# EdoardoBotta/RQ-VAE-Recommender

Hardware: AMD Instinct MI355X
Metric: item-embeddings quantized/sec (RQ-VAE fwd+bwd) (higher is better)
Workload: dtype f32 (MLP GEMMs f16x2-emulated)

## Files before the change

### include/rqhip.h

```cpp
#ifndef RQHIP_H
#define RQHIP_H

#include <stddef.h>
#include <stdint.h>

#ifdef __cplusplus
extern "C" {
#endif

#define RQHIP_VERSION 462

#define RQHIP_OK 0
#define RQHIP_EARG (-1)
#define RQHIP_EUNSUPPORTED (-2)
#define RQHIP_EWORKSPACE (-3)

#define RQHIP_MODE_EVAL 0
#define RQHIP_MODE_STE 1
#define RQHIP_MODE_ROTATION 2
#define RQHIP_MODE_GUMBEL 3

typedef void *rqhip_stream_t;

int rqhip_version(void);
// ... 224 lines not shown
    const float *h_mask;
    const float *w_in;
    int w_in_transposed;
    const float *res0;
    float *res0_out;
    const float *codebooks;
    int L, K, mode;
    float beta;
    int64_t *ids;
    float *emb_sum;
    float *loss;
    float *embs_norm;
    const float *w_out;
    int w_out_transposed;
    int out_epilogue;
    const float *out_mask;
    float *out;
    unsigned *out_row_max;
    unsigned *out_col_max;
} rqhip_seam_args;
int rqhip_rq_seam_supported(int D, int H, int L, int K);
int rqhip_rq_seam(const rqhip_seam_args *args, rqhip_stream_t stream);

int rqhip_linear_small_supported(int64_t M, int N, int Kr);
int rqhip_linear_small_plan(int64_t M, int N, int Kr, int *col_blocks, int *waves);
int rqhip_linear_small(const float *a, const float *w, int w_kn, float *out, int64_t M, int N, int Kr, int epilogue, const float *aux,
                       int col_blocks, int waves, rqhip_stream_t stream);

int rqhip_adamw_step(float *const *p, const float *const *g, float *const *m, float *const *v, const int64_t *numel, int n,
                     float *step, unsigned *scratch, float lr, float beta1, float beta2, float eps, float weight_decay,
                     rqhip_stream_t stream);

#define RQHIP_PROF_RQ_FORWARD 1
#define RQHIP_PROF_RQ_BACKWARD 2
#define RQHIP_PROF_GEMM_SPLIT 3
#define RQHIP_PROF_WGRAD 4
#define RQHIP_PROF_MAXIMA 5
#define RQHIP_PROF_IMAGES 6
#define RQHIP_PROF_SEAM 7
#define RQHIP_PROF_LINEAR_SMALL 8
typedef struct {
    int tag;
    float ms;
    double flops, bytes;
} rqhip_profile_record;
int rqhip_profile_enable(int max_records);
// ... 9 lines not shown
```

### rq-vae-recommender_amd/csrc/wgrad.hip

```cpp
#include "rqhip_common.h"

namespace rqhip {

typedef float wg_f32x16 __attribute__((ext_vector_type(16)));
typedef float wg_f32x4 __attribute__((ext_vector_type(4)));
typedef float wg_f32x2 __attribute__((ext_vector_type(2)));

constexpr int kWgChunk = 32;

struct WgradParams {
    const float *g;
    const float *y;
    const float *x;
    float *gm;
    float *out;
    long long M;
    int N, K;
    int nslab_n, nslab_k, msplit;
    long long n_chunks;
    int pow2;
};

template <int V>
struct VecOf;
// ... 256 lines not shown
    pl.cfg = -1;
    if (N % 256 == 0 && K % 256 == 0) { pl.cfg = 0; pl.Nt = 256; pl.Kt = 256; pl.mc = 32; }
    else if (N % 128 == 0 && K % 256 == 0) { pl.cfg = 1; pl.Nt = 128; pl.Kt = 256; pl.mc = 32; }
    else if (N % 256 == 0 && K % 128 == 0) { pl.cfg = 2; pl.Nt = 256; pl.Kt = 128; pl.mc = 32; }
    else if (N % 32 == 0 && K % 128 == 0) { pl.cfg = 3; pl.Nt = 32; pl.Kt = 128; pl.mc = 64; }
    else if (N % 128 == 0 && K % 32 == 0) { pl.cfg = 4; pl.Nt = 128; pl.Kt = 32; pl.mc = 64; }
    if (pl.cfg < 0) return pl;
    pl.nslab_n = N / pl.Nt;
    pl.nslab_k = K / pl.Kt;
    const long long chunks = (M + kWgChunk - 1) / kWgChunk;
    const int slabs = pl.nslab_n * pl.nslab_k;
    long long ms = cu_count() / slabs;
    if (ms < 1) ms = 1;
    if (ms >= 8) ms &= ~7LL;
    if (chunks <= 4) ms = 1;
    if (ms > chunks) ms = chunks > 0 ? chunks : 1;
    pl.msplit = (int)ms;
    pl.pow2 = 1;
    while (pl.pow2 < pl.msplit) pl.pow2 <<= 1;
    pl.lds = (size_t)2 * pl.mc * (pl.Nt + pl.Kt) * sizeof(float);
    return pl;
}

int wgrad_split_cfg(int N, int K);
int launch_wgrad_split_jobs(int n, const float *const *g, const float *const *x, long long M, const int *N, const int *K, float *const *out,
                            int msplit, const unsigned *const *g_max, const unsigned *const *x_max, int half, hipStream_t s);
int launch_wgrad_split(int cfg, const float *g, const float *y, const float *x, long long M, int N, int K, float *gm, float *out,
                       int nslab_n, int nslab_k, int msplit, const unsigned *g_max, const unsigned *x_max, hipStream_t s);

}

using namespace rqhip;

extern "C" size_t rqhip_linear_wgrad_workspace_bytes(int64_t M, int N, int K) {
    if (M <= 0 || N <= 0 || K <= 0) return 0;
    const WgradPlan pl = wgrad_plan(M, N, K);
    if (pl.cfg < 0 || pl.msplit <= 1) return 16;
    return (size_t)pl.msplit * N * K * sizeof(float);
}

extern "C" int rqhip_linear_wgrad_supported(int N, int K) { return wgrad_plan(1 << 20, N, K).cfg >= 0 ? 1 : 0; }

extern "C" int rqhip_linear_wgrad_plan(int64_t M, int N, int K, int *msplit) {
    const WgradPlan pl = wgrad_plan(M, N, K);
    if (msplit) *msplit = pl.cfg < 0 ? 0 : pl.msplit;
    return pl.cfg;
// ... 69 lines not shown
    }
    WgradParams p;
    p.g = g; p.y = y; p.x = x; p.gm = g_masked;
    p.out = pl.msplit > 1 ? reinterpret_cast<float *>(workspace) : dW;
    p.M = M; p.N = N; p.K = K;
    p.nslab_n = pl.nslab_n; p.nslab_k = pl.nslab_k; p.msplit = pl.msplit;
    p.n_chunks = (M + kWgChunk - 1) / kWgChunk;
    p.pow2 = pl.pow2;
    const bool mask = y != nullptr;
    int rc = 0;
    const int scfg = (flags & RQHIP_WGRAD_FP32) ? -1 : wgrad_split_cfg(N, K);
    profile_begin(s, RQHIP_PROF_WGRAD, 2.0 * (double)M * N * K, 4.0 * (double)M * (N * (1 + (y ? 1 : 0) + (g_masked && y ? 1 : 0)) + K));
    if (scfg >= 0 && scfg == pl.cfg) {
        rc = launch_wgrad_split(scfg, g, y, x, M, N, K, g_masked, p.out, pl.nslab_n, pl.nslab_k, pl.msplit, g_col_max, x_col_max, s);
    } else
    switch (pl.cfg) {
        case 0: rc = wgrad_launch<4, 2, 2, 4, 32>(p, pl, mask, s); break;
        case 1: rc = wgrad_launch<4, 1, 1, 8, 32>(p, pl, mask, s); break;
        case 2: rc = wgrad_launch<2, 2, 4, 2, 32>(p, pl, mask, s); break;
        case 3: rc = wgrad_launch<1, 1, 1, 4, 64>(p, pl, mask, s); break;
        default: rc = wgrad_launch<1, 1, 4, 1, 64>(p, pl, mask, s); break;
    }
    if (rc) { profile_end(s); return rc; }
    if (pl.msplit > 1) {
        const size_t nk4 = (size_t)N * K / 4;
        const int tlog = wgrad_reduce_tlog(nk4, pl.pow2);
        const size_t per_wg = (size_t)256 >> tlog;
        hipLaunchKernelGGL(wgrad_reduce_kernel, dim3((unsigned)((nk4 + per_wg - 1) / per_wg)), dim3(256), 0, s,
                           reinterpret_cast<const float *>(workspace), pl.msplit, pl.pow2, tlog, nk4, dW);
        RQ_CHECK_LAUNCH("wgrad_reduce_kernel");
    }
    profile_end(s);
    return RQHIP_OK;
}

static int wgrad_batch_ranges(long long M, const int *N, const int *K, int n, int *half = nullptr) {
    if (n < 2 || n > 4 || M <= 128 || !N || !K) return 0;
    long long tiles = 0;
    int n_full = 0;
    for (int j = 0; j < n; ++j) {
        if (N[j] <= 0 || K[j] <= 0) return 0;
        const int cfg = wgrad_split_cfg(N[j], K[j]);
        if (cfg < 0) return 0;
        n_full += cfg == 0;
        tiles += (long long)(N[j] / (cfg == 1 ? 128 : 256)) * (K[j] / (cfg == 2 ? 128 : 256));
    }
    if (n_full != 0 && n_full != n) return 0;
    if (half) *half = n_full == 0;
    long long ms = cu_count() / tiles;
    if (ms < 1) return 0;
    if (ms >= 8) ms &= ~7LL;
    const long long chunks = (M + kWgChunk - 1) / kWgChunk;
    if (ms > chunks) ms = chunks;
    return (int)ms;
}

// ... 73 lines not shown
```

### rq-vae-recommender_amd/rqhip/_lib.py

```python
from __future__ import annotations

import ctypes as C
import os
import subprocess

import torch

_CSRC = os.path.join(os.path.dirname(os.path.dirname(os.path.abspath(__file__))), "csrc")
SO_PATH = os.path.join(_CSRC, "librqhip.so")

MODE_EVAL, MODE_STE, MODE_ROTATION, MODE_GUMBEL = 0, 1, 2, 3
FWD_SCAN_FP32, FWD_SCAN_VALU, FWD_NO_COOP_TAIL = 0x1, 0x2, 0x10
WGRAD_FP32 = 0x1
BWD_CBGRAD_MATRIX = 0x1
SPLIT_F16X2, SPLIT_BF16X3 = 0, 1
EPI_STORE, EPI_RELU, EPI_RECON, EPI_MASK = 0, 1, 2, 3
PROF_TAGS = {1: "rq_forward", 2: "rq_backward", 3: "gemm_split", 4: "wgrad", 5: "maxima", 6: "weight_images", 7: "rq_seam", 8: "linear_small"}


class ImageJob(C.Structure):
    _fields_ = [("w", C.c_void_p), ("rows", C.c_int), ("cols", C.c_int), ("transpose", C.c_int), ("arith", C.c_int),
                ("image", C.c_void_p), ("image_bytes", C.c_size_t)]


# ... 98 lines not shown
    "rqhip_linear_wgrad_workspace_bytes": (_sz, [_i64, _int, _int]),
    "rqhip_linear_wgrad": (_int, [_vp, _vp, _vp, _i64, _int, _int, _vp, _vp, _vp, _sz, _vp]),
    "rqhip_linear_wgrad_ex": (_int, [_vp, _vp, _vp, _i64, _int, _int, _vp, _vp, _vp, _sz, C.c_uint, _vp]),
    "rqhip_linear_wgrad_f16": (_int, [_vp, _vp, _vp, _i64, _int, _int, _vp, _vp, _vp, _vp, _vp, _sz, _vp]),
    "rqhip_linear_wgrad_f16_batch_plan": (_int, [_i64, C.POINTER(_int), C.POINTER(_int), _int]),
    "rqhip_linear_wgrad_f16_batch_workspace_bytes": (_sz, [_i64, C.POINTER(_int), C.POINTER(_int), _int]),
    "rqhip_linear_wgrad_f16_batch": (_int, [C.POINTER(WgradJob), _int, _i64, _vp, _sz, _vp]),
    "rqhip_linear_wgrad_jobs_supported": (_int, [_int, _int]),
    "rqhip_linear_wgrad_jobs": (_int, [_vp, _vp, _vp, C.POINTER(_int), C.POINTER(_int), _int, _i64, _vp]),
    "rqhip_gemm_split_supported": (_int, [_int, _int]),
    "rqhip_weight_image_bytes": (_sz, [_int, _int, _int]),
    "rqhip_weight_images": (_int, [C.POINTER(ImageJob), _int, _vp]),
    "rqhip_maxima": (_int, [_vp, _vp, _vp, _i64, _int, _vp, _vp, _vp]),
    "rqhip_gemm_split_ex": (_int, [C.POINTER(GemmArgs), _vp]),
    "rqhip_weight_planes_bytes": (_sz, [_int, _int]),
    "rqhip_weight_planes": (_int, [_vp, _int, _int, _int, _vp, _sz, _vp]),
    "rqhip_gemm_split": (_int, [_vp, _i64, _int, _vp, _int, _int, _vp, _vp]),
    "rqhip_gemm_split_recon_workspace_bytes": (_sz, [_i64, _int]),
    "rqhip_gemm_split_recon": (_int, [_vp, _i64, _int, _vp, _int, _vp, _f32, _vp, _vp, _vp, _sz, _vp]),
    "rqhip_recon_rescale_rows": (_int, [_vp, _i64, _int, _f32, _vp, _vp]),
    "rqhip_recon_rescale_rows_ex": (_int, [_vp, _i64, _int, _f32, _vp, _vp, _int, _vp, _vp]),
    "rqhip_rq_seam_supported": (_int, [_int, _int, _int, _int]),
    "rqhip_rq_seam": (_int, [C.POINTER(SeamArgs), _vp]),
    "rqhip_linear_small_supported": (_int, [_i64, _int, _int]),
    "rqhip_linear_small_plan": (_int, [_i64, _int, _int, C.POINTER(_int), C.POINTER(_int)]),
    "rqhip_linear_small": (_int, [_vp, _vp, _int, _vp, _i64, _int, _int, _int, _vp, _int, _int, _vp]),
    "rqhip_adamw_step": (_int, [_vp, _vp, _vp, _vp, _vp, _int, _vp, _vp, _f32, _f32, _f32, _f32, _f32, _vp]),
    "rqhip_profile_enable": (_int, [_int]),
    "rqhip_profile_select": (_int, [C.c_uint]),
    "rqhip_profile_read": (_int, [C.POINTER(_f32), _int, C.POINTER(_int)]),
    "rqhip_profile_read_tagged": (_int, [C.POINTER(ProfileRecord), _int, C.POINTER(_int)]),
}


class RqHipError(RuntimeError):
    pass


def build(force: bool = False) -> str:
    cmd = ["make", "-C", _CSRC, "-j8"] + (["-B"] if force else [])
    proc = subprocess.run(cmd, stdout=subprocess.PIPE, stderr=subprocess.STDOUT, text=True)
    if proc.returncode != 0:
        raise RqHipError("building librqhip.so failed:\n" + proc.stdout[-4000:])
    return SO_PATH


_lib = None


def load(path: str) -> C.CDLL:
    global _lib
    if not os.path.exists(path):
        raise RqHipError(
            f"{path} not found: build it with `python __graft_entry__.py` or `make -C {_CSRC}`. "
            "The HIP extension is the product path; there is no CPU fallback.")
    handle = C.CDLL(path)
    for name, (res, args) in SIGNATURES.items():
        fn = getattr(handle, name)
        fn.restype, fn.argtypes = res, args
    _lib = handle
    return handle


def lib() -> C.CDLL:
    return _lib if _lib is not None else load(SO_PATH)


def check(rc: int, what: str) -> None:
    if rc != 0:
        msg = lib().rqhip_last_error().decode("utf-8", "replace")
        kind = "HIP error" if rc > 0 else "argument error"
        raise RqHipError(f"{what}: {kind} {rc}: {msg}")
```

### rq-vae-recommender_amd/rqhip/autograd.py

```python
from __future__ import annotations

from typing import Optional

import torch
from torch import Tensor

from . import ops


def _dense(g: Optional[Tensor]) -> Optional[Tensor]:
    if g is None:
        return None
    return g.contiguous()


class RqStackFunction(torch.autograd.Function):

    @staticmethod
    def forward(ctx, res0: Tensor, codebooks: Tensor, mode: int, beta: float, want_levels: bool, grad_sink=None):
        out = ops.rq_forward(res0, codebooks, mode, beta, want_embs=want_levels, want_residuals=want_levels)
        ctx.set_materialize_grads(False)
        ctx.save_for_backward(res0, codebooks, out.ids)
        ctx.mode, ctx.beta, ctx.want_levels, ctx.grad_sink = mode, beta, want_levels, grad_sink
        embs = out.embs if want_levels else res0.new_empty((0,))
# ... 36 lines not shown
        cols = both[:ops.SEAM_H] if want_scales else None
        ctx.bwd_cols = both[ops.SEAM_H:] if (want_scales and torch.is_grad_enabled()) else None
        r = ops.rq_seam(h=h, w_in=w_in.detach(), codebooks=codebooks.detach(), mode=mode, beta=beta, w_out=w_out.detach(),
                        epilogue=_lib.EPI_RELU, want_row_max=want_scales, col_max_out=cols)
        ctx.set_materialize_grads(False)
        ctx.save_for_backward(h, w_in, codebooks, w_out, r.res0, r.ids, r.emb_sum, r.out)
        ctx.mode, ctx.beta, ctx.grad_sink, ctx.want_scales = mode, beta, grad_sink, want_scales
        rmax = r.out_row_max if want_scales else h.new_empty((0,), dtype=torch.int32)
        cmax = cols if want_scales else h.new_empty((0,), dtype=torch.int32)
        ctx.mark_non_differentiable(r.ids, r.embs_norm, rmax, cmax)
        return r.ids, r.loss, r.embs_norm, r.out, rmax, cmax

    @staticmethod
    def backward(ctx, _g_ids, g_loss, _g_norm, g_d, _g_rmax=None, _g_cmax=None):
        from . import linear as _lin
        from .dist import claim_grad_sink
        h, w_in, codebooks, w_out, res0, ids, emb_sum, d = ctx.saved_tensors
        need_h, need_win, need_cb, need_wout = ctx.needs_input_grad[:4]
        g_d, g_loss = _dense(g_d), _dense(g_loss)
        B = h.shape[0]
        jobs = _lin.wgrad_jobs_ok(B, [tuple(w_out.shape), tuple(w_in.shape)])
        pending = []
        gw_out = gw_in = None
        g_es = None
        if g_d is not None:
            g_dm = None
            if need_wout:
                if jobs:
                    g_dm = torch.ops.aten.threshold_backward(g_d, d, 0.0)
                    pending.append(_lin.WgradJob(w_out, g_dm, emb_sum, None, None, claim_grad_sink(w_out)))
                else:
                    sink = claim_grad_sink(w_out)
                    gw, gp, _ = _lin.weight_grad(g_d, d, emb_sum, w_out, out=sink, want_masked=False)
                    gw_out = gw.view_as(gw) if sink is not None else gw
                    g_dm = gp if (gp is not None and gp is not g_d) else None
            if need_h or need_win or need_cb:
                g_es = (_lin.chain_input_grad(g_dm, w_out)[0] if g_dm is not None
                        else _lin.chain_input_grad(g_d, w_out, g_mask=d)[0])
        g_res0 = g_cb = None
        if need_h or need_win or need_cb:
            sink = ctx.grad_sink
            out_cb = None
            if need_cb and sink is not None and tuple(sink.view.shape) == tuple(codebooks.shape) and all(
                    p.grad is None and getattr(p, "_rq_sink_epoch", -1) != sink.owner.epoch for p in sink.params):
                out_cb = sink.view
                for p in sink.params:
                    p._rq_sink_epoch = sink.owner.epoch
            g_res0, g_cb = ops.rq_backward(res0, codebooks, ctx.mode, ctx.beta, ids, g_embsum=g_es, g_loss=g_loss,
                                           need_res0=need_h or need_win, need_codebooks=need_cb, out_g_codebooks=out_cb,
                                           cbgrad=ops.cbgrad_default())
            if out_cb is not None and g_cb is not None:
                g_cb = g_cb.view_as(g_cb)
        g_h = None
        if g_res0 is not None and need_win:
            if jobs:
                pending.append(_lin.WgradJob(w_in, g_res0, h, None, None, claim_grad_sink(w_in)))
            else:
                sink = claim_grad_sink(w_in)
                gw, _, _ = _lin.weight_grad(g_res0, None, h, w_in, out=sink)
                gw_in = gw.view_as(gw) if sink is not None else gw
        for j, gw in zip(pending, _lin.launch_wgrads(pending)):
            gw = gw.view_as(gw) if j.sink is not None else gw
            if j.w is w_out:
                gw_out = gw
            else:
                gw_in = gw
        if g_res0 is not None and need_h:
            cols = None
            if ctx.want_scales:
                cols, ctx.bwd_cols = ctx.bwd_cols, None
                if cols is None:
                    cols = _lin.zeros_i32(ops.SEAM_H, h.device)
            g_h, sc = _lin.chain_input_grad(g_res0, w_in, out_mask=h, want_rows=ctx.want_scales, col_out=cols)
            _lin.handoff_grad(g_h, sc if ctx.want_scales else _lin.Scales())
        return g_h, gw_in, g_cb, gw_out, None, None, None, None

# ... 168 lines not shown
```

### rq-vae-recommender_amd/rqhip/linear.py

```python
from enum import IntEnum
from typing import List, NamedTuple, Optional, Sequence, Tuple

import torch
from torch import Tensor

from . import _lib, ops

SPLIT_MIN_ROWS = 4096
_SPLIT_GEMMS = True
_ARITH = ops.F16X2
_FP32 = -1
_ARITH_NAMES = {"f16x2": ops.F16X2, "bf16x3": ops.BF16X3, "fp32": _FP32}


def use_split_gemms(on: bool = True) -> bool:
    global _SPLIT_GEMMS
    before, _SPLIT_GEMMS = _SPLIT_GEMMS, bool(on)
    return before


def use_arith(name: str) -> str:
    global _ARITH
    before = arith_name()
    _ARITH = _ARITH_NAMES[name]
# ... 267 lines not shown
    return _CHAIN


def chain_forward(x: Tensor, w: Tensor, relu: bool, want_rows: bool = False, col_out: Optional[Tensor] = None):
    x = x if x.is_contiguous() else x.contiguous()
    if tuple(w.shape) == (CHAIN_D, CHAIN_H):
        assert not relu
        return ops.rq_seam(h=x, w_in=w.detach()).res0, Scales()
    r = ops.rq_seam(res0=x, w_out=w.detach(), epilogue=_lib.EPI_RELU if relu else _lib.EPI_STORE, want_row_max=want_rows and f16(),
                    col_max_out=col_out if f16() else None)
    return r.out, Scales(r.out_row_max, col_out if f16() else None)


def chain_input_grad(g: Tensor, w: Tensor, *, g_mask: Optional[Tensor] = None, out_mask: Optional[Tensor] = None, want_rows: bool = False,
                     col_out: Optional[Tensor] = None):
    g = g if g.is_contiguous() else g.contiguous()
    if tuple(w.shape) == (CHAIN_H, CHAIN_D):
        assert out_mask is None
        return ops.rq_seam(h=g, h_mask=g_mask, w_in=w.detach(), w_in_transposed=True).res0, Scales()
    assert g_mask is None
    r = ops.rq_seam(res0=g, w_out=w.detach(), w_out_transposed=True, epilogue=_lib.EPI_MASK if out_mask is not None else _lib.EPI_STORE,
                    out_mask=out_mask, want_row_max=want_rows and f16(), col_max_out=col_out if f16() else None)
    return r.out, Scales(r.out_row_max, col_out if f16() else None)


_SMALL = True


def use_small_kernels(on: bool = True) -> bool:
    global _SMALL
    before, _SMALL = _SMALL, bool(on)
    return before


def small_forward(x: Tensor, w: Tensor, relu: bool) -> Tensor:
    return ops.linear_small(x, w.detach(), epilogue=_lib.EPI_RELU if relu else _lib.EPI_STORE)


def small_input_grad(g: Tensor, w: Tensor, below: Optional[Tensor] = None) -> Tensor:
    return ops.linear_small(g, w.detach(), w_kn=True, epilogue=_lib.EPI_MASK if below is not None else _lib.EPI_STORE, aux=below)


class Route(IntEnum):
    NONE = 0
    LIBRARY = 1
    SPLIT = 2
# ... 147 lines not shown
```

### rq-vae-recommender_amd/rqhip/ops.py

```python
from __future__ import annotations

import ctypes as C
from typing import NamedTuple, Optional

import torch
from torch import Tensor

from . import _lib
from ._lib import MODE_EVAL, MODE_GUMBEL, MODE_ROTATION, MODE_STE, RqHipError, check


def _need_gpu(*tensors: Optional[Tensor]) -> torch.device:
    dev = None
    for t in tensors:
        if t is None:
            continue
        if not t.is_cuda:
            raise RqHipError(
                "rqhip ops need ROCm device tensors (got a %s tensor); the HIP kernels are the only "
                "implementation of this path -- there is no CPU fallback." % t.device.type)
        if dev is None:
            dev = t.device
        elif t.device != dev:
            raise RqHipError(f"tensors on different devices: {dev} vs {t.device}")
# ... 141 lines not shown
    if epilogue == _lib.EPI_MASK and (out_mask is None or tuple(out_mask.shape) != (B, H)):
        raise RqHipError("rq_seam: EPI_MASK needs out_mask [B,128]")
    if col_max_out is not None and (col_max_out.dtype != torch.int32 or col_max_out.numel() != H or not col_max_out.is_contiguous()):
        raise RqHipError("rq_seam: col_max_out must be a contiguous int32 [128] tensor (zeroed by the caller)")
    with torch.cuda.device(dev):
        f = lambda *shape: torch.empty(shape, dtype=torch.float32, device=dev)
        a = _lib.SeamArgs()
        a.B, a.D, a.H = B, D, H
        a.h, a.h_mask, a.w_in, a.w_in_transposed = _ptr(h), _ptr(h_mask), _ptr(w_in), int(bool(w_in_transposed))
        r0 = f(B, D) if (h is not None and want_res0) else None
        a.res0, a.res0_out = _ptr(res0) if h is None else None, _ptr(r0)
        ids = torch.empty((L, B), dtype=torch.int64, device=dev) if L > 0 else None
        es = f(B, D) if (L > 0 and want_emb_sum) else None
        loss = f(B) if (L > 0 and want_loss) else None
        norms = f(B, L) if (L > 0 and want_norm) else None
        a.codebooks, a.L, a.K, a.mode, a.beta = _ptr(codebooks), L, K, int(mode), float(beta)
        a.ids, a.emb_sum, a.loss, a.embs_norm = _ptr(ids), _ptr(es), _ptr(loss), _ptr(norms)
        out = f(B, H) if w_out is not None else None
        rmx = torch.empty((H // 32, B), dtype=torch.int32, device=dev) if (w_out is not None and want_row_max) else None
        a.w_out, a.w_out_transposed, a.out_epilogue = _ptr(w_out), int(bool(w_out_transposed)), int(epilogue)
        a.out_mask, a.out, a.out_row_max, a.out_col_max = _ptr(out_mask), _ptr(out), _ptr(rmx), _ptr(col_max_out if w_out is not None else None)
        check(_lib.lib().rqhip_rq_seam(C.byref(a), _stream()), "rqhip_rq_seam")
    return RqSeamOut(r0, ids, es, loss, norms, out, rmx, col_max_out if w_out is not None else None)


def rq_forward(res0: Tensor, codebooks: Tensor, mode: int, beta: float, *, want_embs: bool = True,
               want_residuals: bool = True, want_emb_sum: bool = True, want_loss: bool = True,
               want_norm: bool = True, want_margin: bool = False, scan: str = "auto",
               coop_tail: bool = True) -> RqForwardOut:
    _need_gpu(res0, codebooks)
    res0, codebooks = _f32c(res0, "res0"), _f32c(codebooks, "codebooks")
    if res0.dim() != 2 or codebooks.dim() != 3 or codebooks.shape[2] != res0.shape[1]:
        raise RqHipError(f"shape mismatch: res0 {tuple(res0.shape)}, codebooks {tuple(codebooks.shape)}")
    B, D = res0.shape
    L, K, _ = codebooks.shape
    dev = res0.device
    with torch.cuda.device(dev):
        l = _lib.lib()
        ids = torch.empty((L, B), dtype=torch.int64, device=dev)
        f = lambda *s: torch.empty(s, dtype=torch.float32, device=dev)
        embs = f(L, B, D) if want_embs else None
        residuals = f(L, B, D) if want_residuals else None
        emb_sum = f(B, D) if want_emb_sum else None
        loss = f(B) if want_loss else None
        norm = f(B, L) if want_norm else None
        margin = f(L, B) if want_margin else None
# ... 1042 lines not shown
```

Baseline: 41.00 million.

## Fuse seam backward input-grad and weight-grad GEMMs into single-pass kernels

Adds two HIP kernels for the RQ seam backward. One computes the decoder-side weight gradient and the input gradient g_es in a single pass over g_d, d and emb_sum. The other does the same for the encoder-side linear, producing g_h, dW_in, and the row/column maxima used for f16 scaling. The reductions of both weight-gradient partials are deferred and merged into one pair-reduce launch, removing separate activation reads and several kernel launches. The cost is fixed 128x32 shape specialisation, fp32 MFMA instead of the split-precision paths, and extra LDS pressure.

```diff
diff --git a/include/rqhip.h b/include/rqhip.h
--- a/include/rqhip.h
+++ b/include/rqhip.h
@@ -270,6 +270,12 @@
 int rqhip_rq_seam_supported(int D, int H, int L, int K);
 int rqhip_rq_seam(const rqhip_seam_args *args, rqhip_stream_t stream);
 
+int rqhip_seam_bwd_supported(int D, int H);
+int rqhip_seam_bwd_out(const float *g_d, const float *d, const float *emb_sum, const float *w_out, int64_t M, float *g_es, float *dW_out,
+                       void *workspace, size_t workspace_bytes, int defer_reduce, rqhip_stream_t stream);
+int rqhip_seam_bwd_in(const float *g_res0, const float *h, const float *w_in, int64_t M, float *g_h, unsigned *row_max, unsigned *col_max,
+                      float *dW_in, void *workspace, size_t workspace_bytes, const void *out_workspace, float *dW_out, rqhip_stream_t stream);
+
 int rqhip_linear_small_supported(int64_t M, int N, int Kr);
 int rqhip_linear_small_plan(int64_t M, int N, int Kr, int *col_blocks, int *waves);
 int rqhip_linear_small(const float *a, const float *w, int w_kn, float *out, int64_t M, int N, int Kr, int epilogue, const float *aux,
diff --git a/rq-vae-recommender_amd/csrc/seam_backward.hip b/rq-vae-recommender_amd/csrc/seam_backward.hip
--- /dev/null
+++ b/rq-vae-recommender_amd/csrc/seam_backward.hip
@@ -0,0 +1,411 @@
+#include <type_traits>
+
+#include "rqhip_common.h"
+
+namespace rqhip {
+
+typedef float sb_f32x16 __attribute__((ext_vector_type(16)));
+typedef float sb_f32x4 __attribute__((ext_vector_type(4)));
+
+constexpr int kSbH = 128, kSbD = 32;
+constexpr int kSbNT = 256;
+constexpr int kSbMC = 128;
+constexpr int kSbWS = kSbH + 4;
+constexpr int kSbNS = kSbD + 4;
+constexpr int kSbChunk = 32;
+constexpr int kSbImg = kSbH * kSbD;
+
+int launch_wgrad_reduce(const float *part, int msplit, int N, int K, float *dW, hipStream_t s);
+int launch_wgrad_reduce_pair(const float *part0, int N0, int K0, float *dW0, const float *part1, int N1, int K1, float *dW1, int msplit,
+                             hipStream_t s);
+
+struct SeamBwdParams {
+    const float *g;
+    const float *y;
+    const float *x;
+    const float *w;
+    float *gx;
+    unsigned *row_max;
+    unsigned *col_max;
+    float *part;
+    long long M, n_chunks;
+    int msplit;
+};
+
+__device__ __forceinline__ void sb_stage_weight(float *img, const float *__restrict__ w, int n_out) {
+    constexpr int kPer = kSbImg / kSbNT;
+    float v[kPer];
+#pragma unroll
+    for (int u = 0; u < kPer; ++u) v[u] = w[threadIdx.x + u * kSbNT];
+#pragma unroll
+    for (int u = 0; u < kPer; ++u) {
+        const int e = threadIdx.x + u * kSbNT;
+        const int n = e % n_out, d = e / n_out;
+        const int kk = d >> 1, hh = d & 1;
+        img[(((kk >> 2) * 2 + hh) * n_out + n) * 4 + (kk & 3)] = v[u];
+    }
+}
+
+__device__ __forceinline__ void sb_row_range(const SeamBwdParams &p, long long &r_begin, long long &r_end) {
+    const int split = blockIdx.x;
+    r_begin = (p.n_chunks * split / p.msplit) * kSbChunk;
+    r_end = (p.n_chunks * (split + 1) / p.msplit) * kSbChunk;
+    if (r_end > p.M) r_end = p.M;
+}
+
+__global__ __launch_bounds__(kSbNT) void seam_bwd_out_kernel(const SeamBwdParams p) {
+    constexpr int G4 = kSbMC * kSbH / 4 / kSbNT, X4 = kSbMC * kSbD / 4 / kSbNT;
+    extern __shared__ __attribute__((aligned(16))) char sb_smem[];
+    float *sG = reinterpret_cast<float *>(sb_smem);
+    float *sX = sG + kSbMC * kSbWS;
+    float *img = sX + kSbMC * kSbD;
+
+    const int tid = threadIdx.x, lane = tid & 63, wave = tid >> 6, il = lane & 31, h = lane >> 5;
+    long long r_begin, r_end;
+    sb_row_range(p, r_begin, r_end);
+    const long long n_stage = (r_end - r_begin + kSbMC - 1) / kSbMC;
+
+    sb_f32x4 rg[G4], ry[G4], rx[X4];
+    const sb_f32x4 zero4 = {0.f, 0.f, 0.f, 0.f};
+    auto fetch = [&](long long c) {
+        const long long row0 = r_begin + c * kSbMC;
+#pragma unroll
+        for (int q = 0; q < G4; ++q) {
+            const int f = tid + q * kSbNT;
+            const long long row = row0 + f / (kSbH / 4);
+            const bool ok = row < r_end;
+            const size_t off = (size_t)(ok ? row : 0) * kSbH + 4 * (f % (kSbH / 4));
+            rg[q] = ok ? *reinterpret_cast<const sb_f32x4 *>(p.g + off) : zero4;
+            ry[q] = ok ? *reinterpret_cast<const sb_f32x4 *>(p.y + off) : zero4;
+        }
+#pragma unroll
+        for (int q = 0; q < X4; ++q) {
+            const int f = tid + q * kSbNT;
+            const long long row = row0 + f / (kSbD / 4);
+            const bool ok = row < r_end;
+            rx[q] = ok ? *reinterpret_cast<const sb_f32x4 *>(p.x + (size_t)(ok ? row : 0) * kSbD + 4 * (f % (kSbD / 4))) : zero4;
+        }
+    };
+    auto stash = [&]() {
+#pragma unroll
+        for (int q = 0; q < G4; ++q) {
+            const int f = tid + q * kSbNT;
+            sb_f32x4 v = rg[q];
+            v.x = ry[q].x <= 0.0f ? 0.0f : v.x;
+            v.y = ry[q].y <= 0.0f ? 0.0f : v.y;
+            v.z = ry[q].z <= 0.0f ? 0.0f : v.z;
+            v.w = ry[q].w <= 0.0f ? 0.0f : v.w;
+            *reinterpret_cast<sb_f32x4 *>(sG + (f / (kSbH / 4)) * kSbWS + 4 * (f % (kSbH / 4))) = v;
+        }
+#pragma unroll
+        for (int q = 0; q < X4; ++q) {
+            const int f = tid + q * kSbNT;
+            *reinterpret_cast<sb_f32x4 *>(sX + 4 * f) = rx[q];
+        }
+    };
+
+    sb_f32x16 acc;
+#pragma unroll
+    for (int r = 0; r < 16; ++r) acc[r] = 0.0f;
+
+    if (n_stage > 0) fetch(0);
+    sb_stage_weight(img, p.w, kSbD);
+    if (n_stage > 0) stash();
+    __syncthreads();
+    for (long long c = 0; c < n_stage; ++c) {
+        const bool more = c + 1 < n_stage;
+        if (more) fetch(c + 1);
+        const long long row0 = r_begin + c * kSbMC;
+        const int rows = (int)(r_end - row0 < kSbMC ? r_end - row0 : kSbMC);
+        const float *gA = sG + wave * 32 + il, *xB = sX + il;
+        auto stage = [&](auto full) {
+            constexpr bool FULL = decltype(full)::value;
+#pragma unroll
+            for (int half = 0; half < kSbMC / 64; ++half) {
+                if (!FULL && half * 64 >= rows) break;
+#pragma unroll
+                for (int s = 0; s < 32; ++s) {
+                    const int r = half * 64 + 2 * s + h;
+                    acc = __builtin_amdgcn_mfma_f32_32x32x2f32(gA[r * kSbWS], xB[r * kSbD], acc, 0, 0, 0);
+                }
+            }
+            if (FULL || wave * 32 < rows) {
+                const sb_f32x4 *rowp = reinterpret_cast<const sb_f32x4 *>(sG + (wave * 32 + il) * kSbWS);
+                float x[kSbH / 2];
+#pragma unroll
+                for (int j = 0; j < kSbH / 4; ++j) {
+                    const sb_f32x4 v = rowp[j];
+                    x[2 * j] = h ? v.y : v.x;
+                    x[2 * j + 1] = h ? v.w : v.z;
+                }
+                const sb_f32x4 *img4 = reinterpret_cast<const sb_f32x4 *>(img);
+                sb_f32x16 ge;
+#pragma unroll
+                for (int r = 0; r < 16; ++r) ge[r] = 0.0f;
+#pragma unroll
+                for (int q = 0; q < kSbH / 8; ++q) {
+                    const sb_f32x4 a = img4[(q * 2 + h) * kSbD + il];
+#pragma unroll
+                    for (int i = 0; i < 4; ++i) ge = __builtin_amdgcn_mfma_f32_32x32x2f32(a[i], x[4 * q + i], ge, 0, 0, 0);
+                }
+                const long long row = row0 + wave * 32 + il;
+                if (FULL || row < r_end) {
+                    sb_f32x4 *dst = reinterpret_cast<sb_f32x4 *>(p.gx + (size_t)row * kSbD + 4 * h);
+#pragma unroll
+                    for (int g = 0; g < 4; ++g) dst[2 * g] = sb_f32x4{ge[4 * g], ge[4 * g + 1], ge[4 * g + 2], ge[4 * g + 3]};
+                }
+            }
+        };
+        if (rows == kSbMC) stage(std::true_type{});
+        else stage(std::false_type{});
+        __syncthreads();
+        if (more) stash();
+        __syncthreads();
+    }
+    float *dst = p.part + (size_t)blockIdx.x * kSbH * kSbD;
+#pragma unroll
+    for (int r = 0; r < 16; ++r) dst[(size_t)(wave * 32 + 8 * (r >> 2) + 4 * h + (r & 3)) * kSbD + il] = acc[r];
+}
+
+__global__ __launch_bounds__(kSbNT) void seam_bwd_in_kernel(const SeamBwdParams p) {
+    constexpr int H4 = kSbMC * kSbH / 4 / kSbNT, N4 = kSbMC * kSbD / 4 / kSbNT;
+    extern __shared__ __attribute__((aligned(16))) char sb_smem[];
+    float *sH = reinterpret_cast<float *>(sb_smem);
+    float *sN = sH + kSbMC * kSbWS;
+    float *img = sN + kSbMC * kSbNS;
+    unsigned *colmax_s = reinterpret_cast<unsigned *>(img + kSbImg);
+
+    const int tid = threadIdx.x, lane = tid & 63, wave = tid >> 6, il = lane & 31, h = lane >> 5;
+    long long r_begin, r_end;
+    sb_row_range(p, r_begin, r_end);
+    const long long n_stage = (r_end - r_begin + kSbMC - 1) / kSbMC;
+
+    sb_f32x4 rh[H4], rn[N4];
+    const sb_f32x4 zero4 = {0.f, 0.f, 0.f, 0.f};
+    auto fetch = [&](long long c) {
+        const long long row0 = r_begin + c * kSbMC;
+#pragma unroll
+        for (int q = 0; q < H4; ++q) {
+            const int f = tid + q * kSbNT;
+            const long long row = row0 + f / (kSbH / 4);
+            const bool ok = row < r_end;
+            rh[q] = ok ? *reinterpret_cast<const sb_f32x4 *>(p.y + (size_t)(ok ? row : 0) * kSbH + 4 * (f % (kSbH / 4))) : zero4;
+        }
+#pragma unroll
+        for (int q = 0; q < N4; ++q) {
+            const int f = tid + q * kSbNT;
+            const long long row = row0 + f / (kSbD / 4);
+            const bool ok = row < r_end;
+            rn[q] = ok ? *reinterpret_cast<const sb_f32x4 *>(p.g + (size_t)(ok ? row : 0) * kSbD + 4 * (f % (kSbD / 4))) : zero4;
+        }
+    };
+    unsigned cmx[4] = {0u, 0u, 0u, 0u};
+    auto swap_stage = [&](long long c, bool write_out, bool stash) {
+        const long long row0 = r_begin + c * kSbMC;
+#pragma unroll
+        for (int q = 0; q < H4; ++q) {
+            const int f = tid + q * kSbNT;
+            const int r = f / (kSbH / 4), c4 = f % (kSbH / 4);
+            sb_f32x4 *slot = reinterpret_cast<sb_f32x4 *>(sH + r * kSbWS + 4 * c4);
+            if (write_out && row0 + r < r_end) {
+                const sb_f32x4 v = *slot;
+                *reinterpret_cast<sb_f32x4 *>(p.gx + (size_t)(row0 + r) * kSbH + 4 * c4) = v;
+                const float vc[4] = {v.x, v.y, v.z, v.w};
+#pragma unroll
+                for (int j = 0; j < 4; ++j) {
+                    const unsigned bits = __builtin_bit_cast(unsigned, vc[j]) & 0x7fffffffu;
+                    cmx[j] = bits > cmx[j] ? bits : cmx[j];
+                }
+            }
+            if (stash) *slot = rh[q];
+        }
+        if (stash) {
+#pragma unroll
+            for (int q = 0; q < N4; ++q) {
+                const int f = tid + q * kSbNT;
+                *reinterpret_cast<sb_f32x4 *>(sN + (f / (kSbD / 4)) * kSbNS + 4 * (f % (kSbD / 4))) = rn[q];
+            }
+        }
+    };
+
+    sb_f32x16 acc;
+#pragma unroll
+    for (int r = 0; r < 16; ++r) acc[r] = 0.0f;
+
+    if (n_stage > 0) fetch(0);
+    if (tid < kSbH) colmax_s[tid] = 0u;
+    sb_stage_weight(img, p.w, kSbH);
+    if (n_stage > 0) swap_stage(0, false, true);
+    __syncthreads();
+    const int blk = wave;
+    for (long long c = 0; c < n_stage; ++c) {
+        const bool more = c + 1 < n_stage;
+        if (more) fetch(c + 1);
+        const long long row0 = r_begin + c * kSbMC;
+        const int rows = (int)(r_end - row0 < kSbMC ? r_end - row0 : kSbMC);
+        const float *gA = sN + il, *xB = sH + blk * 32 + il;
+        const sb_f32x4 *img4 = reinterpret_cast<const sb_f32x4 *>(img);
+        auto tiles = [&](auto full) {
+            constexpr bool FULL = decltype(full)::value;
+#pragma unroll
+            for (int t = 0; t < kSbMC / 32; ++t) {
+                if (!FULL && (t & ~1) * 32 >= rows) break;
+#pragma unroll
+                for (int s = 0; s < 16; ++s) {
+                    const int r = t * 32 + 2 * s + h;
+                    acc = __builtin_amdgcn_mfma_f32_32x32x2f32(gA[r * kSbNS], xB[r * kSbWS], acc, 0, 0, 0);
+                }
+                if (!FULL && t * 32 >= rows) continue;
+                const sb_f32x4 *rowp = reinterpret_cast<const sb_f32x4 *>(sN + (t * 32 + il) * kSbNS);
+                float es[kSbD / 2];
+#pragma unroll
+                for (int j = 0; j < kSbD / 4; ++j) {
+                    const sb_f32x4 v = rowp[j];
+                    es[2 * j] = h ? v.y : v.x;
+                    es[2 * j + 1] = h ? v.w : v.z;
+                }
+                sb_f32x16 gh;
+#pragma unroll
+                for (int r = 0; r < 16; ++r) gh[r] = 0.0f;
+#pragma unroll
+                for (int q = 0; q < kSbD / 8; ++q) {
+                    const sb_f32x4 a = img4[(q * 2 + h) * kSbH + 32 * blk + il];
+#pragma unroll
+                    for (int i = 0; i < 4; ++i) gh = __builtin_amdgcn_mfma_f32_32x32x2f32(a[i], es[4 * q + i], gh, 0, 0, 0);
+                }
+                const long long row = row0 + t * 32 + il;
+                const bool row_ok = FULL || row < r_end;
+                float *slot = sH + (t * 32 + il) * kSbWS + 32 * blk + 4 * h;
+                unsigned rmx = 0u;
+#pragma unroll
+                for (int g = 0; g < 4; ++g) {
+                    sb_f32x4 v = {gh[4 * g], gh[4 * g + 1], gh[4 * g + 2], gh[4 * g + 3]};
+                    const sb_f32x4 m = *reinterpret_cast<const sb_f32x4 *>(slot + 8 * g);
+                    v.x = m.x <= 0.0f ? 0.0f : v.x; v.y = m.y <= 0.0f ? 0.0f : v.y;
+                    v.z = m.z <= 0.0f ? 0.0f : v.z; v.w = m.w <= 0.0f ? 0.0f : v.w;
+                    *reinterpret_cast<sb_f32x4 *>(slot + 8 * g) = v;
+                    const float vc[4] = {v.x, v.y, v.z, v.w};
+#pragma unroll
+                    for (int cc = 0; cc < 4; ++cc) {
+                        const unsigned bits = __builtin_bit_cast(unsigned, vc[cc]) & 0x7fffffffu;
+                        rmx = bits > rmx ? bits : rmx;
+                    }
+                }
+                if (p.row_max) {
+                    const unsigned o = (unsigned)shfl_xor32((int)rmx);
+                    rmx = o > rmx ? o : rmx;
+                    if (row_ok && h == 0) p.row_max[(size_t)blk * p.M + row] = rmx;
+                }
+            }
+        };
+        if (rows == kSbMC) tiles(std::true_type{});
+        else tiles(std::false_type{});
+        __syncthreads();
+        swap_stage(c, true, more);
+        __syncthreads();
+    }
+    float *dst = p.part + (size_t)blockIdx.x * kSbH * kSbD;
+#pragma unroll
+    for (int r = 0; r < 16; ++r) dst[(size_t)(8 * (r >> 2) + 4 * h + (r & 3)) * kSbH + 32 * blk + il] = acc[r];
+    if (p.col_max) {
+#pragma unroll
+        for (int j = 0; j < 4; ++j)
+            if (cmx[j]) atomicMax(&colmax_s[4 * (tid & 31) + j], cmx[j]);
+        __syncthreads();
+        if (tid < kSbH && colmax_s[tid]) atomicMax(p.col_max + tid, colmax_s[tid]);
+    }
+}
+
+constexpr size_t kSbOutLds = (size_t)(kSbMC * kSbWS + kSbMC * kSbD + kSbImg) * sizeof(float);
+constexpr size_t kSbInLds = (size_t)(kSbMC * kSbWS + kSbMC * kSbNS + kSbImg + kSbH) * sizeof(float);
+
+static bool sb_al16(const void *q) { return (reinterpret_cast<uintptr_t>(q) & 15u) == 0; }
+
+static int sb_ranges(int64_t M, int N, int K) {
+    int msplit = 0;
+    const int cfg = rqhip_linear_wgrad_plan(M, N, K, &msplit);
+    return (cfg == 3 || cfg == 4) ? msplit : 0;
+}
+
+}
+
+using namespace rqhip;
+
+extern "C" int rqhip_seam_bwd_supported(int D, int H) { return (D == kSbD && H == kSbH) ? 1 : 0; }
+
+static size_t sb_workspace_bytes(int64_t M) { return rqhip_linear_wgrad_workspace_bytes(M, kSbH, kSbD); }
+
+extern "C" int rqhip_seam_bwd_out(const float *g_d, const float *d, const float *emb_sum, const float *w_out, int64_t M, float *g_es,
+                                  float *dW_out, void *workspace, size_t workspace_bytes, int defer_reduce, rqhip_stream_t stream) {
+    if (M < 4096 || !g_d || !d || !emb_sum || !w_out || !g_es || !dW_out) {
+        set_error("seam_bwd_out: null pointer or fewer than 4096 rows (M = %lld)", (long long)M);
+        return M >= 0 && M < 4096 ? RQHIP_EUNSUPPORTED : RQHIP_EARG;
+    }
+    if (!sb_al16(g_d) || !sb_al16(d) || !sb_al16(emb_sum) || !sb_al16(w_out) || !sb_al16(g_es) || !sb_al16(dW_out) || !sb_al16(workspace)) {
+        set_error("seam_bwd_out: pointers must be 16-byte aligned");
+        return RQHIP_EARG;
+    }
+    const int msplit = sb_ranges(M, kSbH, kSbD);
+    if (msplit < 1) {
+        set_error("seam_bwd_out: no weight-gradient plan for 128 x 32");
+        return RQHIP_EUNSUPPORTED;
+    }
+    if (msplit > 1 && (!workspace || workspace_bytes < sb_workspace_bytes(M))) {
+        set_error("seam_bwd_out: workspace too small (rqhip_linear_wgrad_workspace_bytes(M, 128, 32))");
+        return RQHIP_EWORKSPACE;
+    }
+    hipStream_t s = reinterpret_cast<hipStream_t>(stream);
+    SeamBwdParams p;
+    p.g = g_d; p.y = d; p.x = emb_sum; p.w = w_out; p.gx = g_es; p.row_max = nullptr; p.col_max = nullptr;
+    p.part = msplit > 1 ? reinterpret_cast<float *>(workspace) : dW_out;
+    p.M = M; p.n_chunks = (M + kSbChunk - 1) / kSbChunk; p.msplit = msplit;
+    static LdsGrant grant;
+    RQ_RETURN_IF_HIP(grant.ensure(reinterpret_cast<const void *>(seam_bwd_out_kernel), 160 * 1024));
+    profile_begin(s, RQHIP_PROF_SEAM, 4.0 * (double)M * kSbH * kSbD, 4.0 * (double)M * (2 * kSbH + 2 * kSbD));
+    hipLaunchKernelGGL(seam_bwd_out_kernel, dim3(msplit), dim3(kSbNT), kSbOutLds, s, p);
+    profile_end(s);
+    RQ_CHECK_LAUNCH("seam_bwd_out_kernel");
+    if (msplit > 1 && !defer_reduce) return launch_wgrad_reduce(p.part, msplit, kSbH, kSbD, dW_out, s);
+    return RQHIP_OK;
+}
+
+extern "C" int rqhip_seam_bwd_in(const float *g_res0, const float *h, const float *w_in, int64_t M, float *g_h, unsigned *row_max,
+                                 unsigned *col_max, float *dW_in, void *workspace, size_t workspace_bytes, const void *out_workspace,
+                                 float *dW_out, rqhip_stream_t stream) {
+    if (M < 4096 || !g_res0 || !h || !w_in || !g_h || !dW_in || ((out_workspace != nullptr) != (dW_out != nullptr))) {
+        set_error("seam_bwd_in: null pointer, fewer than 4096 rows (M = %lld), or only one of out_workspace / dW_out", (long long)M);
+        return M >= 0 && M < 4096 ? RQHIP_EUNSUPPORTED : RQHIP_EARG;
+    }
+    if (!sb_al16(g_res0) || !sb_al16(h) || !sb_al16(w_in) || !sb_al16(g_h) || !sb_al16(dW_in) || !sb_al16(workspace) ||
+        !sb_al16(out_workspace) || !sb_al16(dW_out)) {
+        set_error("seam_bwd_in: pointers must be 16-byte aligned");
+        return RQHIP_EARG;
+    }
+    const int msplit = sb_ranges(M, kSbD, kSbH);
+    if (msplit < 1 || (out_workspace && sb_ranges(M, kSbH, kSbD) != msplit)) {
+        set_error("seam_bwd_in: no weight-gradient plan for 32 x 128 (or another number of row ranges than the deferred 128 x 32 blocks)");
+        return RQHIP_EUNSUPPORTED;
+    }
+    if (msplit > 1 && (!workspace || workspace_bytes < sb_workspace_bytes(M))) {
+        set_error("seam_bwd_in: workspace too small (rqhip_linear_wgrad_workspace_bytes(M, 128, 32))");
+        return RQHIP_EWORKSPACE;
+    }
+    hipStream_t s = reinterpret_cast<hipStream_t>(stream);
+    SeamBwdParams p;
+    p.g = g_res0; p.y = h; p.x = nullptr; p.w = w_in; p.gx = g_h; p.row_max = row_max; p.col_max = col_max;
+    p.part = msplit > 1 ? reinterpret_cast<float *>(workspace) : dW_in;
+    p.M = M; p.n_chunks = (M + kSbChunk - 1) / kSbChunk; p.msplit = msplit;
+    static LdsGrant grant;
+    RQ_RETURN_IF_HIP(grant.ensure(reinterpret_cast<const void *>(seam_bwd_in_kernel), 160 * 1024));
+    profile_begin(s, RQHIP_PROF_SEAM, 4.0 * (double)M * kSbH * kSbD, 4.0 * (double)M * (2 * kSbH + kSbD + (row_max ? 4 : 0)));
+    hipLaunchKernelGGL(seam_bwd_in_kernel, dim3(msplit), dim3(kSbNT), kSbInLds, s, p);
+    profile_end(s);
+    RQ_CHECK_LAUNCH("seam_bwd_in_kernel");
+    if (msplit > 1) {
+        if (out_workspace)
+            return launch_wgrad_reduce_pair(reinterpret_cast<const float *>(out_workspace), kSbH, kSbD, dW_out, p.part, kSbD, kSbH, dW_in,
+                                            msplit, s);
+        return launch_wgrad_reduce(p.part, msplit, kSbD, kSbH, dW_in, s);
+    }
+    return RQHIP_OK;
+}
diff --git a/rq-vae-recommender_amd/csrc/wgrad.hip b/rq-vae-recommender_amd/csrc/wgrad.hip
--- a/rq-vae-recommender_amd/csrc/wgrad.hip
+++ b/rq-vae-recommender_amd/csrc/wgrad.hip
@@ -302,6 +302,47 @@
     return pl;
 }
 
+static int wgrad_reduce_go(const float *part, int msplit, int N, int K, float *dW, hipStream_t s) {
+    int pow2 = 1;
+    while (pow2 < msplit) pow2 <<= 1;
+    const size_t nk4 = (size_t)N * K / 4;
+    const int tlog = wgrad_reduce_tlog(nk4, pow2);
+    const size_t per_wg = (size_t)256 >> tlog;
+    hipLaunchKernelGGL(wgrad_reduce_kernel, dim3((unsigned)((nk4 + per_wg - 1) / per_wg)), dim3(256), 0, s, part, msplit, pow2, tlog, nk4, dW);
+    RQ_CHECK_LAUNCH("wgrad_reduce_kernel");
+    return 0;
+}
+
+int launch_wgrad_reduce(const float *part, int msplit, int N, int K, float *dW, hipStream_t s) {
+    profile_begin(s, RQHIP_PROF_WGRAD, 0.0, 4.0 * (double)N * K * (msplit + 1));
+    const int rc = wgrad_reduce_go(part, msplit, N, K, dW, s);
+    profile_end(s);
+    return rc;
+}
+
+int launch_wgrad_reduce_pair(const float *part0, int N0, int K0, float *dW0, const float *part1, int N1, int K1, float *dW1, int msplit,
+                             hipStream_t s) {
+    WgradReduceJobs rj;
+    rj.n = 2; rj.msplit = msplit; rj.pow2 = 1;
+    while (rj.pow2 < msplit) rj.pow2 <<= 1;
+    const float *part[2] = {part0, part1};
+    float *dw[2] = {dW0, dW1};
+    const size_t nk4[2] = {(size_t)N0 * K0 / 4, (size_t)N1 * K1 / 4};
+    unsigned blocks = 0;
+    for (int j = 0; j < 4; ++j) {
+        const int i = j < 2 ? j : 0;
+        rj.part[j] = part[i]; rj.dw[j] = dw[i]; rj.nk4[j] = nk4[i]; rj.tlog[j] = wgrad_reduce_tlog(nk4[i], rj.pow2);
+        rj.first[j] = blocks;
+        const size_t per_wg = (size_t)256 >> rj.tlog[j];
+        if (j < 2) blocks += (unsigned)((nk4[i] + per_wg - 1) / per_wg);
+    }
+    profile_begin(s, RQHIP_PROF_WGRAD, 0.0, 4.0 * (double)(N0 * K0 + N1 * K1) * (msplit + 1));
+    hipLaunchKernelGGL(wgrad_reduce_jobs_kernel, dim3(blocks), dim3(256), 0, s, rj);
+    profile_end(s);
+    RQ_CHECK_LAUNCH("wgrad_reduce_jobs_kernel");
+    return 0;
+}
+
 int wgrad_split_cfg(int N, int K);
 int launch_wgrad_split_jobs(int n, const float *const *g, const float *const *x, long long M, const int *N, const int *K, float *const *out,
                             int msplit, const unsigned *const *g_max, const unsigned *const *x_max, int half, hipStream_t s);
@@ -417,16 +458,9 @@
         default: rc = wgrad_launch<1, 1, 4, 1, 64>(p, pl, mask, s); break;
     }
     if (rc) { profile_end(s); return rc; }
-    if (pl.msplit > 1) {
-        const size_t nk4 = (size_t)N * K / 4;
-        const int tlog = wgrad_reduce_tlog(nk4, pl.pow2);
-        const size_t per_wg = (size_t)256 >> tlog;
-        hipLaunchKernelGGL(wgrad_reduce_kernel, dim3((unsigned)((nk4 + per_wg - 1) / per_wg)), dim3(256), 0, s,
-                           reinterpret_cast<const float *>(workspace), pl.msplit, pl.pow2, tlog, nk4, dW);
-        RQ_CHECK_LAUNCH("wgrad_reduce_kernel");
-    }
+    if (pl.msplit > 1) rc = wgrad_reduce_go(reinterpret_cast<const float *>(workspace), pl.msplit, N, K, dW, s);
     profile_end(s);
-    return RQHIP_OK;
+    return rc;
 }
 
 static int wgrad_batch_ranges(long long M, const int *N, const int *K, int n, int *half = nullptr) {
diff --git a/rq-vae-recommender_amd/rqhip/_lib.py b/rq-vae-recommender_amd/rqhip/_lib.py
--- a/rq-vae-recommender_amd/rqhip/_lib.py
+++ b/rq-vae-recommender_amd/rqhip/_lib.py
@@ -144,6 +144,9 @@
     "rqhip_recon_rescale_rows_ex": (_int, [_vp, _i64, _int, _f32, _vp, _vp, _int, _vp, _vp]),
     "rqhip_rq_seam_supported": (_int, [_int, _int, _int, _int]),
     "rqhip_rq_seam": (_int, [C.POINTER(SeamArgs), _vp]),
+    "rqhip_seam_bwd_supported": (_int, [_int, _int]),
+    "rqhip_seam_bwd_out": (_int, [_vp, _vp, _vp, _vp, _i64, _vp, _vp, _vp, _sz, _int, _vp]),
+    "rqhip_seam_bwd_in": (_int, [_vp, _vp, _vp, _i64, _vp, _vp, _vp, _vp, _vp, _sz, _vp, _vp, _vp]),
     "rqhip_linear_small_supported": (_int, [_i64, _int, _int]),
     "rqhip_linear_small_plan": (_int, [_i64, _int, _int, C.POINTER(_int), C.POINTER(_int)]),
     "rqhip_linear_small": (_int, [_vp, _vp, _int, _vp, _i64, _int, _int, _int, _vp, _int, _int, _vp]),
@@ -155,6 +158,9 @@
 }
 
 
+NEWER = ("rqhip_seam_bwd_supported", "rqhip_seam_bwd_out", "rqhip_seam_bwd_in")
+
+
 class RqHipError(RuntimeError):
     pass
 
@@ -177,7 +183,10 @@
             f"{path} not found: build it with `python __graft_entry__.py` or `make -C {_CSRC}`. "
             "The HIP extension is the product path; there is no CPU fallback.")
     handle = C.CDLL(path)
+    other = os.path.realpath(path) != os.path.realpath(SO_PATH)
     for name, (res, args) in SIGNATURES.items():
+        if other and name in NEWER and not hasattr(handle, name):
+            continue
         fn = getattr(handle, name)
         fn.restype, fn.argtypes = res, args
     _lib = handle
@@ -186,6 +195,10 @@
 
 def lib() -> C.CDLL:
     return _lib if _lib is not None else load(SO_PATH)
+
+
+def has(name: str) -> bool:
+    return name not in NEWER or hasattr(lib(), name)
 
 
 def check(rc: int, what: str) -> None:
diff --git a/rq-vae-recommender_amd/rqhip/autograd.py b/rq-vae-recommender_amd/rqhip/autograd.py
--- a/rq-vae-recommender_amd/rqhip/autograd.py
+++ b/rq-vae-recommender_amd/rqhip/autograd.py
@@ -82,8 +82,15 @@
         jobs = _lin.wgrad_jobs_ok(B, [tuple(w_out.shape), tuple(w_in.shape)])
         pending = []
         gw_out = gw_in = None
+        fused = (not jobs and g_d is not None and need_h and need_win and need_cb and need_wout
+                 and _lin.seam_backward_ok(B, (g_d, d, emb_sum, h, res0)))
+        out_pending = None
         g_es = None
-        if g_d is not None:
+        if fused:
+            sink = claim_grad_sink(w_out)
+            g_es, gw, out_pending = ops.seam_bwd_out(g_d, d, emb_sum, w_out.detach(), out=sink, defer_reduce=True)
+            gw_out = gw.view_as(gw) if sink is not None else gw
+        elif g_d is not None:
             g_dm = None
             if need_wout:
                 if jobs:
@@ -112,6 +119,19 @@
             if out_cb is not None and g_cb is not None:
                 g_cb = g_cb.view_as(g_cb)
         g_h = None
+        if fused:
+            sink = claim_grad_sink(w_in)
+            cols = None
+            if ctx.want_scales:
+                cols, ctx.bwd_cols = ctx.bwd_cols, None
+                if cols is None:
+                    cols = _lin.zeros_i32(ops.SEAM_H, h.device)
+            scaled = ctx.want_scales and _lin.f16()
+            g_h, rmx, gw = ops.seam_bwd_in(g_res0, h, w_in.detach(), out=sink, want_row_max=scaled, col_max_out=cols if scaled else None,
+                                           pending=out_pending)
+            gw_in = gw.view_as(gw) if sink is not None else gw
+            _lin.handoff_grad(g_h, _lin.Scales(rmx, cols if scaled else None) if ctx.want_scales else _lin.Scales())
+            return g_h, gw_in, g_cb, gw_out, None, None, None, None
         if g_res0 is not None and need_win:
             if jobs:
                 pending.append(_lin.WgradJob(w_in, g_res0, h, None, None, claim_grad_sink(w_in)))
diff --git a/rq-vae-recommender_amd/rqhip/linear.py b/rq-vae-recommender_amd/rqhip/linear.py
--- a/rq-vae-recommender_amd/rqhip/linear.py
+++ b/rq-vae-recommender_amd/rqhip/linear.py
@@ -313,6 +313,20 @@
     r = ops.rq_seam(res0=g, w_out=w.detach(), w_out_transposed=True, epilogue=_lib.EPI_MASK if out_mask is not None else _lib.EPI_STORE,
                     out_mask=out_mask, want_row_max=want_rows and f16(), col_max_out=col_out if f16() else None)
     return r.out, Scales(r.out_row_max, col_out if f16() else None)
+
+
+_SEAM_BACKWARD = True
+
+
+def use_seam_backward(on: bool = True) -> bool:
+    global _SEAM_BACKWARD
+    before, _SEAM_BACKWARD = _SEAM_BACKWARD, bool(on)
+    return before
+
+
+def seam_backward_ok(rows: int, operands: Sequence[Tensor]) -> bool:
+    return bool(_SEAM_BACKWARD and rows >= ops.SEAM_BWD_MIN_ROWS and ops.seam_bwd_supported(CHAIN_D, CHAIN_H)
+                and all(dense_f32(t) for t in operands))
 
 
 _SMALL = True
diff --git a/rq-vae-recommender_amd/rqhip/ops.py b/rq-vae-recommender_amd/rqhip/ops.py
--- a/rq-vae-recommender_amd/rqhip/ops.py
+++ b/rq-vae-recommender_amd/rqhip/ops.py
@@ -187,6 +187,68 @@
         a.out_mask, a.out, a.out_row_max, a.out_col_max = _ptr(out_mask), _ptr(out), _ptr(rmx), _ptr(col_max_out if w_out is not None else None)
         check(_lib.lib().rqhip_rq_seam(C.byref(a), _stream()), "rqhip_rq_seam")
     return RqSeamOut(r0, ids, es, loss, norms, out, rmx, col_max_out if w_out is not None else None)
+
+
+SEAM_BWD_MIN_ROWS = 4096
+
+
+def seam_bwd_supported(D: int, H: int) -> bool:
+    return bool(_lib.has("rqhip_seam_bwd_supported") and _lib.lib().rqhip_seam_bwd_supported(int(D), int(H)))
+
+
+class SeamBwdPending(NamedTuple):
+    workspace: Tensor
+    dw: Tensor
+    rows: int
+
+
+def _seam_bwd_out_tensor(out: Optional[Tensor], shape, dev, what: str) -> Tensor:
+    if out is not None and (tuple(out.shape) != shape or out.dtype != torch.float32 or not out.is_contiguous()):
+        raise RqHipError(f"{what}: `out` must be a contiguous float32 {list(shape)} tensor")
+    return out if out is not None else torch.empty(shape, dtype=torch.float32, device=dev)
+
+
+def seam_bwd_out(g_d: Tensor, d: Tensor, emb_sum: Tensor, w_out: Tensor, *, out: Optional[Tensor] = None, defer_reduce: bool = False):
+    _need_gpu(g_d, d, emb_sum, w_out, out)
+    g_d, d, emb_sum, w_out = _f32c(g_d, "g_d"), _f32c(d, "d"), _f32c(emb_sum, "emb_sum"), _f32c(w_out, "w_out")
+    M = g_d.shape[0]
+    if tuple(g_d.shape) != (M, SEAM_H) or d.shape != g_d.shape or tuple(emb_sum.shape) != (M, 32) or tuple(w_out.shape) != (SEAM_H, 32):
+        raise RqHipError(f"seam_bwd_out: shapes g_d {tuple(g_d.shape)}, d {tuple(d.shape)}, emb_sum {tuple(emb_sum.shape)}, w_out {tuple(w_out.shape)}")
+    dev = g_d.device
+    with torch.cuda.device(dev):
+        l = _lib.lib()
+        dw = _seam_bwd_out_tensor(out, (SEAM_H, 32), dev, "seam_bwd_out")
+        g_es = torch.empty((M, 32), dtype=torch.float32, device=dev)
+        wsb = l.rqhip_linear_wgrad_workspace_bytes(M, SEAM_H, 32)
+        ws = torch.empty((max(wsb, 16),), dtype=torch.uint8, device=dev)
+        check(l.rqhip_seam_bwd_out(_ptr(g_d), _ptr(d), _ptr(emb_sum), _ptr(w_out), M, _ptr(g_es), _ptr(dw), _ptr(ws), wsb,
+                                   1 if defer_reduce else 0, _stream()), "rqhip_seam_bwd_out")
+    return g_es, dw, (SeamBwdPending(ws, dw, M) if defer_reduce else None)
+
+
+def seam_bwd_in(g_res0: Tensor, h: Tensor, w_in: Tensor, *, out: Optional[Tensor] = None, want_row_max: bool = False,
+                col_max_out: Optional[Tensor] = None, pending: Optional[SeamBwdPending] = None):
+    _need_gpu(g_res0, h, w_in, out, col_max_out)
+    g_res0, h, w_in = _f32c(g_res0, "g_res0"), _f32c(h, "h"), _f32c(w_in, "w_in")
+    M = h.shape[0]
+    if tuple(h.shape) != (M, SEAM_H) or tuple(g_res0.shape) != (M, 32) or tuple(w_in.shape) != (32, SEAM_H):
+        raise RqHipError(f"seam_bwd_in: shapes g_res0 {tuple(g_res0.shape)}, h {tuple(h.shape)}, w_in {tuple(w_in.shape)}")
+    if col_max_out is not None and (col_max_out.dtype != torch.int32 or col_max_out.numel() != SEAM_H or not col_max_out.is_contiguous()):
+        raise RqHipError("seam_bwd_in: col_max_out must be a contiguous int32 [128] tensor (zeroed by the caller)")
+    if pending is not None and pending.rows != M:
+        raise RqHipError("seam_bwd_in: the pending decoder-side blocks were formed over another number of rows")
+    dev = h.device
+    with torch.cuda.device(dev):
+        l = _lib.lib()
+        dw = _seam_bwd_out_tensor(out, (32, SEAM_H), dev, "seam_bwd_in")
+        g_h = torch.empty((M, SEAM_H), dtype=torch.float32, device=dev)
+        rmx = torch.empty((SEAM_H // 32, M), dtype=torch.int32, device=dev) if want_row_max else None
+        wsb = l.rqhip_linear_wgrad_workspace_bytes(M, 32, SEAM_H)
+        ws = torch.empty((max(wsb, 16),), dtype=torch.uint8, device=dev)
+        check(l.rqhip_seam_bwd_in(_ptr(g_res0), _ptr(h), _ptr(w_in), M, _ptr(g_h), _ptr(rmx), _ptr(col_max_out), _ptr(dw), _ptr(ws), wsb,
+                                  _ptr(pending.workspace) if pending is not None else None, _ptr(pending.dw) if pending is not None else None,
+                                  _stream()), "rqhip_seam_bwd_in")
+    return g_h, rmx, dw
 
 
 def rq_forward(res0: Tensor, codebooks: Tensor, mode: int, beta: float, *, want_embs: bool = True,
```

Result: no change. 41.21 million (median of 6 runs) (+0.5%).
